# WilliamYi96/HGR-Net

Hardware: AMD Instinct MI355X
Metric: images/sec over 21K-class hierarchy, batch 512; hit@1 parity vs reference (higher is better)
Workload: dtype f16

## Files before the change

### hgr-net_amd/_lib.py

```python
from __future__ import annotations

import ctypes as C
import os
from pathlib import Path

import torch

_HERE = Path(__file__).resolve().parent
LIB_PATH = Path(os.environ.get("HGR_LIB", _HERE / "lib" / "libhgr.so"))

HGR_BF16, HGR_F16 = 0, 1
EPI_NONE, EPI_BIAS, EPI_BIAS_QUICKGELU, EPI_BIAS_RESIDUAL, EPI_BIAS_RELU, EPI_BIAS_ADD16_RELU, EPI_ACCUM, EPI_QGELU_GRAD16 = 0, 1, 2, 3, 4, 5, 6, 7

_p, _i, _l, _f = C.c_void_p, C.c_int, C.c_int64, C.c_float

SIGNATURES = {
    "hgr_gemm_nt": [_p, _l, _p, _l, _p, _l, _p, _p, _l, _i, _i, _i, _i, _i, _i, _p],
    "hgr_gemm_set_tile": [_i],
    "hgr_gemm_set_tail": [_i, _i],
    "hgr_gemm_set_persist": [_i],
    "hgr_gemm_set_ws": [_i],
    "hgr_gemm_set_p8": [_i],
    "hgr_im2col_patches": [_p, _p, _i, _i, _i, _i, _i, _p],
    "hgr_im2col_patches_ex": [_p, _p, _i, _i, _i, _i, _i, _i, _i, _p],
# ... 47 lines not shown
    "hgr_gemm_tn_splitk": [_p, _l, _p, _l, _p, _l, _i, _i, _i, _i, _i, _p],
    "hgr_gemm_tn_tile": [_i, _i],
    "hgr_conv3x3_wgrad_splitk": [_p, _l, _p, _p, _l, _i, _i, _i, _i, _i, _i, _i, _p],
    "hgr_relu_bwd16": [_p, _p, _p, _l, _i, _p],
    "hgr_add16": [_p, _p, _p, _l, _i, _p],
    "hgr_avgpool2_bwd_nhwc": [_p, _p, _i, _i, _i, _i, _i, _p],
    "hgr_attnpool_tokens_bwd": [_p, _p, _i, _i, _i, _i, _p],
    "hgr_im2col3x3_t": [_p, _p, _i, _i, _i, _i, _l, _i, _p],
    "hgr_bn_fold": [_p, _p, _p, _p, _p, _f, _p, _p, _i, _i, _i, _i, _i, _p],
    "hgr_bn_unfold_grad": [_p, _l, _p, _p, _p, _p, _p, _f, _p, _p, _p, _i, _i, _i, _p],
    "hgr_csr_group_aggregate": [_p, _l, _p, _p, _p, _p, _i, _p, _p, _p, _p, _i, _p, _p, _p, _p, _i, _p, _p, _l, _i, _f, _i, _p],
    "hgr_gemm_nt_res_stats": [_p, _l, _p, _l, _p, _p, _l, _p, _p, _i, _i, _i, _i, _p],
    "hgr_vit_head": [_p, _p, _l, _l, _p, _p, _f, _p, _p, _i, _i, _i, _i, _p],
    "hgr_gemm_nt_res_stats_guard": [_p, _l, _p, _l, _p, _p, _l, _p, _p, _f, _p, _i, _i, _i, _i, _p],
    "hgr_gemm_nt_ln": [_p, _l, _p, _l, _p, _l, _p, _p, _p, _f, _i, _i, _i, _i, _i, _p],
    "hgr_gemm_nt_ln_mha": [_p, _l, _p, _l, _p, _p, _p, _f, _p, _l, _i, _i, _i, _i, _i, _p],
    "hgr_gemm_nt_bias_gelu_dual": [_p, _l, _p, _l, _p, _l, _p, _l, _p, _i, _i, _i, _i, _p],
    "hgr_gemm_nt_qgelu_grad_colsum": [_p, _l, _p, _l, _p, _l, _p, _l, _p, _i, _i, _i, _i, _p],
    "hgr_vit_embed_ln_stats": [_p, _p, _p, _p, _p, _p, _p, _p, _i, _i, _i, _f, _i, _p],
    "hgr_row_stats16": [_p, _p, _p, _p, _i, _i, _i, _p],
    "hgr_pair_rows_f32": [_p, _p, _p, _i, _i, _l, _p, _i, _p],
    "hgr_logits_eval_workspace_bytes": [_i, _i],
    "hgr_logits_eval": [_p, _p, _i, _i, _i, _p, _p, _p, _i, _p, _p, _i, _p, _i, _i, _p, _p, _p, _p, _i, _p],
    "hgr_logits_eval_tile_stage": [_p, _p, _i, _i, _i, _p, _p, _p, _i, _p, _p, _i, _p, _i, _i, _p, _p, _p, _p, _i, _p],
    "hgr_logits_eval_row_stage": [_p, _p, _i, _i, _i, _p, _p, _p, _i, _p, _p, _i, _p, _i, _i, _p, _p, _p, _p, _i, _p],
    "hgr_comm_unique_id": [_p],
    "hgr_comm_init": [_i, _i, _p],
    "hgr_comm_destroy": [],
    "hgr_comm_rank": [],
    "hgr_comm_world": [],
# ... 60 lines not shown
```

### hgr-net_amd/clip/model.py

```python
from __future__ import annotations

import os
from collections import OrderedDict
from typing import Dict, Optional, Tuple, Union

import numpy as np
import torch
from torch import nn

from .. import ops
from .._lib import (EPI_BIAS, EPI_BIAS_ADD16_RELU, EPI_BIAS_QUICKGELU, EPI_BIAS_RELU, EPI_BIAS_RESIDUAL, EPI_NONE,
                    HgrError)


class QuickGELU(nn.Module):
    """Placeholder so ``mlp`` keeps the reference's child names (c_fc, gelu, c_proj); the activation
    itself is fused into the c_fc GEMM epilogue (HGR_EPI_BIAS_QUICKGELU)."""


class ResidualAttentionBlock(nn.Module):
    def __init__(self, d_model: int, n_head: int):
        super().__init__()
        self.attn = nn.MultiheadAttention(d_model, n_head)
        self.ln_1 = nn.LayerNorm(d_model)
# ... 117 lines not shown
    def get(self, name: str, shape, dtype, device) -> torch.Tensor:
        n = int(np.prod(shape))
        t = self._b.get(name)
        if t is None or t.numel() < n or t.dtype != dtype or t.device != device:
            t = torch.empty(n, dtype=dtype, device=device)
            self._b[name] = t
            self.epoch += 1
        return t[:n].view(*shape)


IMG_STREAMS = max(1, int(os.environ.get("HGR_IMG_STREAMS", "1")))
IMG_STREAMS_MIN_ROWS = 8192
CLS_LAST = os.environ.get("HGR_CLS_LAST", "1") != "0"
LN_FUSED = os.environ.get("HGR_LN_FUSED", "1") != "0"
QKV_MHA = os.environ.get("HGR_QKV_MHA", "1") != "0"


def ln_fusable(w: int, m: int = 0) -> bool:
    return LN_FUSED and w % 128 == 0 and m * 4 * w * 2 < 2 ** 32


def _run_blocks(x: Optional[torch.Tensor], blocks, heads: int, b: int, l: int, causal: bool, dt: torch.dtype, ws: _Workspace, tag: str,
                taps: Optional[dict] = None, tap_prefix: str = "", pair=None, stats: Optional[torch.Tensor] = None,
                flag: Optional[torch.Tensor] = None, cls_only_last: bool = False):
    m, w = (pair[0] if pair is not None else x).shape
    dev = (pair[0] if pair is not None else x).device
    qkv = ws.get(tag + ".qkv", (m, 3 * w), dt, dev)
    att = ws.get(tag + ".att", (m, w), dt, dev)
    u16 = ws.get(tag + ".u16", (m, 4 * w), dt, dev)
    if pair is not None:
# ... 11 lines not shown
                ops.gemm_nt_ln(ch, k.wf_in[:w], qkv.view(b, l, 3 * w)[:, 0, :w], k.s_in[:w], k.c_in[:w], st_q, k.eps1, tag="q_cls")
            elif fused_attn:
                ops.gemm_nt_ln_mha(xh, k.wf_in, att, k.s_in, k.c_in, stats, b, l, heads, causal, k.eps1)
            else:
                ops.gemm_nt_ln(xh, k.wf_in, qkv, k.s_in, k.c_in, stats, k.eps1, tag="qkv")
            if not fused_attn:
                ops.mha(qkv, att, b, l, heads, causal, q_rows=1 if last_cls else 0)
            if last_cls:
                ca = att.view(b, l, w)[:, 0, :]
                st_c = ws.get(tag + ".stats_cls", (b, w // 64, 2), torch.float32, dev)
                u_c = ws.get(tag + ".u16_cls", (b, 4 * w), dt, dev)
                ops.gemm_nt_res_stats(ca, k.w_out, ch, cl, k.b_out, st_c, tag="out_cls", flag=flag)
                ops.gemm_nt_ln(ch, k.wf_fc, u_c, k.s_fc, k.c_fc, st_c, k.eps2, quickgelu=True, tag="fc_cls")
                ops.gemm_nt_res_stats(u_c, k.w_proj, ch, cl, k.b_proj, st_c, tag="proj_cls", flag=flag)
                break
            ops.gemm_nt_res_stats(att, k.w_out, xh, xl, k.b_out, stats, tag="out", flag=flag)
            ops.gemm_nt_ln(xh, k.wf_fc, u16, k.s_fc, k.c_fc, stats, k.eps2, quickgelu=True, tag="fc")
            ops.gemm_nt_res_stats(u16, k.w_proj, xh, xl, k.b_proj, stats, tag="proj", flag=flag)
            if taps is not None:
                taps[f"{tap_prefix}.resblocks.{i}"] = ops.pair_value(xh, xl).view(b, l, w)
        return None
    h16 = ws.get(tag + ".h16", (m, w), dt, dev)
    for i, k in enumerate(blocks):
        ops.layernorm(x, k.ln1[0], k.ln1[1], h16)
        ops.gemm_nt(h16, k.w_in, qkv, bias=k.b_in, epilogue=EPI_BIAS)
        ops.mha(qkv, att, b, l, heads, causal)
        ops.gemm_nt(att, k.w_out, x, bias=k.b_out, residual=x, epilogue=EPI_BIAS_RESIDUAL)
        ops.layernorm(x, k.ln2[0], k.ln2[1], h16)
        ops.gemm_nt(h16, k.w_fc, u16, bias=k.b_fc, epilogue=EPI_BIAS_QUICKGELU)
        ops.gemm_nt(u16, k.w_proj, x, bias=k.b_proj, residual=x, epilogue=EPI_BIAS_RESIDUAL)
        if taps is not None:
            taps[f"{tap_prefix}.resblocks.{i}"] = x.view(b, l, w).clone()
    return x
# ... 407 lines not shown
```

### hgr-net_amd/csrc/hgr_common.h

```cpp
#pragma once
#include <hip/hip_runtime.h>
#include <stdint.h>
#include <stdio.h>
#include <stdarg.h>
#include <stdlib.h>

#include "../../include/hgr.h"

#define HGR_WAVE 64

#ifdef HGR_LAB
#define HGR_LAB_ON(expr) (expr)
static inline int hgr_lab_env(const char *name) { const char *e = getenv(name); return e ? atoi(e) : 0; }
#else
#define HGR_LAB_ON(expr) false
static inline int hgr_lab_env(const char *) { return 0; }
#endif

typedef __attribute__((ext_vector_type(8))) __bf16 bf16x8;
typedef __attribute__((ext_vector_type(8))) _Float16 f16x8;
typedef __attribute__((ext_vector_type(4))) __bf16 bf16x4;
typedef __attribute__((ext_vector_type(4))) _Float16 f16x4;
typedef __attribute__((ext_vector_type(4))) float f32x4;
typedef __attribute__((ext_vector_type(16))) float f32x16;
typedef __attribute__((ext_vector_type(4))) unsigned int u32x4;
typedef __attribute__((ext_vector_type(2))) unsigned int u32x2;

#define AS1 __attribute__((address_space(1)))
#define AS3 __attribute__((address_space(3)))

template <int DT> struct T16;
template <> struct T16<HGR_BF16> {
    typedef __bf16 elem;
    typedef bf16x8 vec8;
    typedef bf16x4 vec4;
    static __device__ __forceinline__ f32x4 mfma16(vec8 a, vec8 b, f32x4 c) {
        return __builtin_amdgcn_mfma_f32_16x16x32_bf16(a, b, c, 0, 0, 0);
    }
    static __device__ __forceinline__ f32x16 mfma32(vec8 a, vec8 b, f32x16 c) {
        return __builtin_amdgcn_mfma_f32_32x32x16_bf16(a, b, c, 0, 0, 0);
    }
};
template <> struct T16<HGR_F16> {
    typedef _Float16 elem;
// ... 136 lines not shown
```

### hgr-net_amd/csrc/hgr_gemm.hip

```cpp
#include "hgr_gemm_common.h"

using namespace hgr_gemm;

int hgr_conv3x3_c32_launch(const void *x, const void *w, const float *bias, void *out, int B, int H, int W, int Cout, int Kp,
                           int dtype, int relu, void *stream, int pool, int C);

namespace {
constexpr int BM = 128, BN = 128;

int duo_group_env() {
    static int g = -1;
    if (g < 0) { const char *e = getenv("HGR_GEMM_GROUP"); g = e ? atoi(e) : 0; if (g < 0) g = 0; }
    return g;
}
int duo_group() { return duo_group_env() ? duo_group_env() : 4; }
int duo_group_for(int tiles_n) { return duo_group_env() ? duo_group_env() : (tiles_n <= 8 ? 1 : 4); }
int duo_dbg() {
    static int d = -1;
    if (d < 0) d = hgr_lab_env("HGR_GEMM_DBG");
    return d;
}

struct DuoPlan { int big_panels, nbig, tiles_m_half, grid; };
int tail_env = -2, pb_env = -2;
// ... 353 lines not shown
        HGR_CHECK_LAUNCH("hgr_gemm_nt_ln");
        return HGR_OK;
    }
    if (ws_enabled() && hgr_gemm_force_tile() == 0 && ws_covers(M, N, K, WS_LNC)) {
        launch_ws(a, dtype, WS_LNC, act, false, (hipStream_t)stream);
        HGR_CHECK_LAUNCH("hgr_gemm_nt_ln");
        return HGR_OK;
    }
    dim3 grid;
    duo_apply_plan(a, true, grid);
    launch_duo(a, dtype, act ? HGR_EPI_BIAS_QUICKGELU : HGR_EPI_BIAS, false, 2, grid, (hipStream_t)stream);
    HGR_CHECK_LAUNCH("hgr_gemm_nt_ln");
    return HGR_OK;
}

extern "C" int hgr_gemm_nt_bias_gelu_dual(const void *A, int64_t lda, const void *W, int64_t ldw, void *pre, int64_t ldpre, void *post, int64_t ldpost,
                                          const float *bias, int M, int N, int K, int dtype, void *stream) {
    if (int rc = ln_common_checks("hgr_gemm_nt_bias_gelu_dual", A, lda, W, ldw, M, N, K, dtype)) return rc;
    HGR_REQUIRE(pre && post && bias, "hgr_gemm_nt_bias_gelu_dual: null pre / post / bias");
    HGR_REQUIRE(ldpre >= N && ldpost >= N && ldpre % 8 == 0 && ldpost % 8 == 0 && ldpre < (1 << 23) && ldpost < (1 << 23) && hgr_aligned(pre, 16) && hgr_aligned(post, 16) && hgr_aligned(bias, 16),
                "hgr_gemm_nt_bias_gelu_dual: pre / post / bias must be 16-byte aligned, leading dimensions >= N, %% 8 == 0, < 2^23");
    GemmArgs a;
    ln_args(a, A, lda, W, ldw, pre, ldpre, M, N, K);
    a.bias = bias; a.ln_xh = post; a.ln_ldx = ldpost;
    dim3 grid;
    duo_apply_plan(a, true, grid);
    launch_duo(a, dtype, HGR_EPI_BIAS, false, 4, grid, (hipStream_t)stream);
    HGR_CHECK_LAUNCH("hgr_gemm_nt_bias_gelu_dual");
    return HGR_OK;
}
// ... 68 lines not shown
```

### hgr-net_amd/csrc/hgr_gemm_common.h

```cpp
#pragma once
#include "hgr_common.h"
#include <stdlib.h>
#include <type_traits>

namespace hgr_gemm {

constexpr int BK = 64;

struct GemmArgs {
    const char *A; int64_t lda;
    const char *W; int64_t ldw;
    void *C; int64_t ldc;
    const float *bias;
    const float *res; int64_t ldr;
    int M, N, K;
    int tiles_m, tiles_n;
    int m_fastest;
    int vec_ok;
    int dbg;
    int cH, cW, cC, cStride, cHo, cWo;
    unsigned cMagic;
    int cUni;
    int kc; int64_t csplit;
    float *ln_stats; int ln_slots; float ln_eps;
// ... 206 lines not shown
        if constexpr (DW > 0) __builtin_amdgcn_sched_group_barrier(0x200, DW, 0);
        if constexpr (DV > 0) __builtin_amdgcn_sched_group_barrier(0x020, DV, 0);
        mfma16_interleave_step<NR, NW, NV, M_ + 1, NM>();
    }
}
template <int NR, int NW, int NV>
__device__ __forceinline__ void mfma16_interleave() { mfma16_interleave_step<NR, NW, NV, 0>(); }
template <int NR, int NW, int NV>
__device__ __forceinline__ void mfma8_interleave() { mfma16_interleave_step<NR, NW, NV, 0, 8>(); }

enum { V128_PLAIN = 0, V128_TALL = 1, V128_CONV = 2, V128_CONV_TALL = 3 };
void launch_128(const GemmArgs &a, int dtype, int epi, bool out32, int variant, dim3 grid, hipStream_t s);
void launch_256(const GemmArgs &a, int dtype, int epi, bool out32, bool conv, dim3 grid, hipStream_t s);
void launch_duo(const GemmArgs &a, int dtype, int epi, bool out32, int ln, dim3 grid, hipStream_t s);
int duo_set_persist(int enabled);
enum { WS_PLAIN = 0, WS_LNC = 1, WS_LNP = 2 };
bool ws_covers(int M, int N, int K, int mode);
void launch_ws(const GemmArgs &a, int dtype, int mode, int act, bool hasb, hipStream_t s);
int ws_enabled();
int ws_set(int enabled);
bool p8_covers(int M, int N, int K);
void launch_p8(const GemmArgs &a, int dtype, int act, hipStream_t s);
bool p8_wanted(int M, int N, int K);
int p8_set(int mode);

struct SlabArgs {
    const char *A; int64_t lda;
    const char *W; int64_t ldw;
    int M, K, Np;
    const int *tpos, *epos;
// ... 9 lines not shown
```

### hgr-net_amd/csrc/hgr_gemm_duo.hip

```cpp
#include "hgr_gemm_common.h"

namespace hgr_gemm {

#ifndef HGR_PAIR_V2
#define HGR_PAIR_V2 1
#endif
constexpr int NTD = 256;
constexpr int DUO_A0 = 0, DUO_A1 = 32768, DUO_W0 = 65536, DUO_W1 = 73728, DUO_LDS = 81920;

__device__ __forceinline__ void store16_sc1(void *ptr, u32x4 v) {
    asm volatile("global_store_dwordx4 %0, %1, off sc1\n\ts_nop 1" ::"v"(ptr), "v"(v) : "memory");
}

template <int DT, int EPI, bool OUT32, int LN, int MH, bool CONV = false>
__device__ __forceinline__ void duo_tile(const GemmArgs &p, char *smem, const int m0, const int n0) {
    typedef typename T16<DT>::vec8 vec8;
    typedef typename T16<DT>::elem E;
    constexpr int WR = 64 * MH;
    int tid = threadIdx.x;
    if (LN == 1) asm volatile("" : "+v"(tid));
    const int lane = tid & 63;
    const int wave = __builtin_amdgcn_readfirstlane(tid >> 6);
    const int wm = wave >> 1, wn = wave & 1;
    const int r = lane & 15, g = lane >> 4;

    unsigned oA0[4], oA1[4], oW0[2], oW1[2];
    unsigned vA0[CONV ? 4 : 1], vA1[CONV ? 4 : 1];
#pragma unroll
    for (int i = 0; i < 4; ++i) {
        const int id = (i * 4 + wave) * 64 + lane;
        const int pr = id >> 3, c = (id & 7) ^ (pr & 7);
        const int ra = MH == 2 ? (pr >> 6) * 128 + (pr & 63) : pr;
        if (CONV) {
#pragma unroll
            for (int half = 0; half < 2; ++half) {
// ... 82 lines not shown
                for (int i = 0; i < p.ln_slots / 2; ++i) { const f32x4 t = sp[i]; s1 += t[0] + t[2]; s2 += t[1] + t[3]; }
        }
        return ln_finalize(s1, s2, 1.0f / (float)p.K, p.ln_eps);
    };
    const int nk = p.K / 64;
    const int offA = (wm * 64 + r) * 128;
    const int offW = (wn * 32 + r) * 128;
    const int sw0 = ((0 + g) ^ (r & 7)) * 16, sw1 = ((4 + g) ^ (r & 7)) * 16;
    vec8 af[4][2], wf0[2][2], wf1[2][2];
#ifndef HGR_DUO_PF
#define HGR_DUO_PF 2
#endif
#ifndef HGR_DUO_PF_DMA_FIRST
#define HGR_DUO_PF_DMA_FIRST 0
#endif
    constexpr bool PF_BUILD = HGR_DUO_PF == 1 || (HGR_DUO_PF == 2 && LN == 2);
    const bool pf_tile = MH == 2 && !CONV && PF_BUILD && m0 + 256 <= p.M && n0 + 128 <= p.N && (p.K & 127) == 0 && p.K >= 256;
    if (pf_tile) {
      if constexpr (MH == 2 && !CONV && PF_BUILD) {
        vec8 afB[4][2];
        auto &afA = af;
        auto rdW = [&](vec8 (&wf)[2][2], int base) {
#pragma unroll
            for (int j = 0; j < 2; ++j) {
                wf[j][0] = *(const vec8 *)(smem + base + offW + j * 2048 + sw0);
                wf[j][1] = *(const vec8 *)(smem + base + offW + j * 2048 + sw1);
            }
        };
        auto rdA = [&](vec8 (&a)[4][2], int base) {
#pragma unroll
            for (int i = 0; i < 4; ++i) {
// ... 288 lines not shown
            const unsigned gl = (unsigned)rr * ldgB + ch * 16;
#pragma unroll
            for (int q = 0; q < 8 * MH; ++q) {
                const u32x4 v = *(const u32x4 *)(my + (q * 8 + rr) * RS + ch * 16);
                *(u32x4 *)(cw + (cl + q * 8 * ldcB)) = v;
                const vec8 h = __builtin_bit_cast(vec8, v);
                vec8 o;
#pragma unroll
                for (int e = 0; e < 8; ++e) o[e] = quick_gelu_train16<DT>((float)h[e]);
                *(u32x4 *)(gw + (gl + q * 8 * ldgB)) = __builtin_bit_cast(u32x4, o);
            }
            return;
        }
#pragma unroll
        for (int q = 0; q < 8 * MH; ++q)
            *(u32x4 *)(cw + (cl + q * 8 * ldcB)) = *(const u32x4 *)(my + (q * 8 + rr) * RS + ch * 16);
        return;
    }
    if (full && !OUT32 && epi_has_idn16(EPI) && (p.ldc & 7) == 0 && (p.ldr & 7) == 0 && (reinterpret_cast<uintptr_t>(p.C) & 15) == 0 && (reinterpret_cast<uintptr_t>(p.res) & 15) == 0) {
        constexpr int RS = 272;
        char *my = smem + wave * (32 * RS);
        f32x4 bq[2][2];
#pragma unroll
        for (int b = 0; b < 2; ++b)
#pragma unroll
            for (int j = 0; j < 2; ++j) bq[b][j] = HAS_BIAS ? *(const f32x4 *)(p.bias + n0 + wn * 64 + b * 32 + j * 16 + g * 4) : (f32x4){0.f, 0.f, 0.f, 0.f};
        const int r8 = lane >> 3, c8 = lane & 7;
        const int64_t wrow = m0 + wm * WR, wcol = n0 + wn * 64;
        char *cw = (char *)p.C + (wrow * p.ldc + wcol) * 2;
        const char *iw = (const char *)p.res + (wrow * p.ldr + wcol) * 2;
        const unsigned ldcB = (unsigned)p.ldc * 2u, ldiB = (unsigned)p.ldr * 2u;
// ... 120 lines not shown
                        v[e + 4] = (hi4[e] + b8hi[e]) + pair_dec<DT>(oh[e + 4], (ol[1] >> (8 * e)) & 255u);
                    }
#endif
#if HGR_PAIR_V2
                    u32x4 nh;
                    u32x2 nl;
                    {
                        unsigned tq[8];
#pragma unroll
                        for (int e2 = 0; e2 < 4; ++e2) nh[e2] = pair_split2<DT>(v[2 * e2], v[2 * e2 + 1], tq[2 * e2], tq[2 * e2 + 1]);
                        unsigned n0, n1;
                        pair_put_q<DT, 0>(n0, tq[0]); pair_put_q<DT, 1>(n0, tq[1]); pair_put_q<DT, 2>(n0, tq[2]); pair_put_q<DT, 3>(n0, tq[3]);
                        pair_put_q<DT, 0>(n1, tq[4]); pair_put_q<DT, 1>(n1, tq[5]); pair_put_q<DT, 2>(n1, tq[6]); pair_put_q<DT, 3>(n1, tq[7]);
                        nl = (u32x2){n0, n1};
                    }
                    *(u32x4 *)(hw + (xo + (rl + q * 8) * ldxB)) = nh;
#else
                    vec8 nh;
                    u32x2 nl = (u32x2){0u, 0u};
#pragma unroll
                    for (int e = 0; e < 4; ++e) {
                        unsigned q0, q1;
                        E h0, h1;
                        pair_split<DT>(v[e], h0, q0);
                        pair_split<DT>(v[e + 4], h1, q1);
                        nh[e] = h0; nh[e + 4] = h1;
                        nl[0] |= q0 << (8 * e);
                        nl[1] |= q1 << (8 * e);
                    }
                    *(u32x4 *)(hw + (xo + (rl + q * 8) * ldxB)) = __builtin_bit_cast(u32x4, nh);
#endif
                    if (!HGR_LAB_ON(p.dbg & 64)) *(u32x2 *)(lw + (lo8 + (rl + q * 8) * ldlB)) = nl;
                    s1[q] = ((v[0] + v[1]) + (v[2] + v[3])) + ((v[4] + v[5]) + (v[6] + v[7]));
                    s2[q] = (__builtin_fmaf(v[0], v[0], v[1] * v[1]) + __builtin_fmaf(v[2], v[2], v[3] * v[3])) +
                            (__builtin_fmaf(v[4], v[4], v[5] * v[5]) + __builtin_fmaf(v[6], v[6], v[7] * v[7]));
                }
                if (HGR_LAB_ON(p.dbg & 32)) continue;
#define HGR_DPP_STAGE8(CTRL) _Pragma("unroll") for (int q = 0; q < 2; ++q) { \
                    s1[q] += __builtin_bit_cast(float, __builtin_amdgcn_update_dpp(0, __builtin_bit_cast(int, s1[q]), CTRL, 0xF, 0xF, true)); \
                    s2[q] += __builtin_bit_cast(float, __builtin_amdgcn_update_dpp(0, __builtin_bit_cast(int, s2[q]), CTRL, 0xF, 0xF, true)); }
                HGR_DPP_STAGE8(0xB1) HGR_DPP_STAGE8(0x4E) HGR_DPP_STAGE8(0x141)
#undef HGR_DPP_STAGE8
                if (c8 == 0) {
#pragma unroll
                    for (int q = 0; q < 2; ++q) {
                        *(float2 *)(sw + (so + (rl + q * 8) * ldsB)) = make_float2(s1[q], s2[q]);
                        gbits = max(gbits, __float_as_uint(s2[q]));
                    }
                }
            }
            if (p.ln_flag && gbits > __float_as_uint(p.ln_guard)) atomicMax(p.ln_flag, gbits);
            return;
        }
        const float *addp = EPI == HGR_EPI_ACCUM ? (const float *)p.C : p.res;
        const int64_t ldadd = EPI == HGR_EPI_ACCUM ? p.ldc : p.ldr;
        char *cw = (char *)p.C + (wrow * p.ldc + wcol) * 4;
        const char *aw = (const char *)addp + (wrow * ldadd + wcol) * 4;
        const unsigned ldcB = (unsigned)p.ldc * 4u, ldaB = (unsigned)ldadd * 4u;
        const unsigned cl = rq * ldcB + cq * 16, al = rq * ldaB + cq * 16;
#pragma unroll
        for (int a = 0; a < MH; ++a)
// ... 33 lines not shown
        lnrow[tid] = ln_row_stats();
        __syncthreads();
#pragma unroll
        for (int a = 0; a < MH; ++a)
#pragma unroll
        for (int i = 0; i < 4; ++i) {
            const int m = m0 + wm * WR + a * 64 + i * 16 + r;
            const float2 mr = lnrow[wm * WR + a * 64 + i * 16 + r];
            if (m >= p.M) continue;
#pragma unroll
            for (int b = 0; b < 2; ++b)
#pragma unroll
            for (int j = 0; j < 2; ++j) {
                const int n = n0 + wn * 64 + b * 32 + j * 16 + g * 4;
                const f32x4 sq = *(const f32x4 *)(p.ln_s + n), cq4 = *(const f32x4 *)(p.ln_c + n);
                *(u32x2 *)((E *)p.C + (int64_t)m * p.ldc + n) = ln_out16<DT, EPI == HGR_EPI_BIAS_QUICKGELU>(mr, acc[a][b][i][j], sq, cq4);
            }
        }
        return;
    }
    if (LN == 1) {
        typedef typename T16<DT>::vec4 hvec4;
        constexpr int RS = 272;
        char *my = smem + wave * (32 * RS);
        const int rq = lane >> 4, cq = lane & 15;
#pragma unroll
        for (int a = 0; a < MH; ++a)
#pragma unroll
        for (int ih = 0; ih < 2; ++ih) {
            const int row0 = m0 + wm * WR + a * 64 + ih * 32;
#pragma unroll
// ... 11 lines not shown
                const bool ok = row < p.M;
                const int64_t at = row * p.ln_ldx + n0 + wn * 64 + cq * 4;
                if (ok) {
                    const hvec4 oh = *(const hvec4 *)((const E *)p.ln_xh + at);
                    const unsigned ol = *(const unsigned *)((const unsigned char *)p.ln_xl + at);
#pragma unroll
                    for (int e = 0; e < 4; ++e) v[e] += pair_dec<DT>(oh[e], (ol >> (8 * e)) & 255u);
                }
                const float s1 = row16_sum((v[0] + v[1]) + (v[2] + v[3]));
                const float s2 = row16_sum(__builtin_fmaf(v[0], v[0], v[1] * v[1]) + __builtin_fmaf(v[2], v[2], v[3] * v[3]));
                if (ok) {
                    hvec4 nh;
                    unsigned nl = 0u;
#pragma unroll
                    for (int e = 0; e < 4; ++e) { unsigned q; E h; pair_split<DT>(v[e], h, q); nh[e] = h; nl |= q << (8 * e); }
                    *(hvec4 *)((E *)p.ln_xh + at) = nh;
                    *(unsigned *)((unsigned char *)p.ln_xl + at) = nl;
                    if (cq == 0) *(float2 *)(p.ln_stats + (row * p.ln_slots + (n0 >> 6) + wn) * 2) = make_float2(s1, s2);
                    if (cq == 0 && p.ln_flag && __float_as_uint(s2) > __float_as_uint(p.ln_guard)) atomicMax(p.ln_flag, __float_as_uint(s2));
                }
            }
        }
        return;
    }
    if (LN == 4) {
#pragma unroll
        for (int a = 0; a < MH; ++a)
#pragma unroll
        for (int i = 0; i < 4; ++i) {
            const int m = m0 + wm * WR + a * 64 + i * 16 + r;
            if (m >= p.M) continue;
#pragma unroll
            for (int b = 0; b < 2; ++b)
// ... 94 lines not shown
        const int per = GROUP * p.tiles_n, grp = wg / per, first = grp * GROUP;
        const int gs = min(GROUP, tiles_m - first), loc = wg - grp * per;
        tm = first + loc % gs; tn = loc / gs;
    }
    if (half) duo_tile<DT, EPI, OUT32, LN, 1, CONV>(p, smem, p.big_panels * 256 + tm * 128, tn * 128);
    else duo_tile<DT, EPI, OUT32, LN, 2, CONV>(p, smem, tm * 256, tn * 128);
  };
    if constexpr (PERSIST) {
        for (int vb = (int)blockIdx.x; vb < total; vb += (int)gridDim.x) {
            one_tile(vb);
            if (vb + (int)gridDim.x < total) HGR_RBAR();
        }
    } else one_tile((int)blockIdx.x);
}

namespace {
template <int DT>
void launch_duo_dt(const GemmArgs &a, int epi, bool out32, int ln, dim3 grid, hipStream_t s) {
    switch (ln) {
        case 1: hipLaunchKernelGGL((gemm_nt_duo<DT, HGR_EPI_BIAS_RESIDUAL, true, 1>), grid, dim3(NTD), 0, s, a); return;
        case 2:
            if (epi == HGR_EPI_BIAS_QUICKGELU) hipLaunchKernelGGL((gemm_nt_duo<DT, HGR_EPI_BIAS_QUICKGELU, false, 2>), grid, dim3(NTD), 0, s, a);
            else hipLaunchKernelGGL((gemm_nt_duo<DT, HGR_EPI_BIAS, false, 2>), grid, dim3(NTD), 0, s, a);
            return;
        case 4: hipLaunchKernelGGL((gemm_nt_duo<DT, HGR_EPI_BIAS, false, 4>), grid, dim3(NTD), 0, s, a); return;
        case 5: hipLaunchKernelGGL((gemm_nt_duo<DT, HGR_EPI_BIAS_RELU, false, 0, true>), grid, dim3(NTD), 0, s, a); return;
        default: break;
    }
#define HGR_DUO(E) do { if (out32) hipLaunchKernelGGL((gemm_nt_duo<DT, E, true>), grid, dim3(NTD), 0, s, a); \
                        else hipLaunchKernelGGL((gemm_nt_duo<DT, E, false>), grid, dim3(NTD), 0, s, a); } while (0)
// ... 26 lines not shown
        n &= ~7;
        if (n < 8) n = 8;
    }
    return n;
}

void launch_duo(const GemmArgs &a0, int dtype, int epi, bool out32, int ln, dim3 grid, hipStream_t s) {
    GemmArgs a = a0;
    a.total = 0;
    const int ds = duo_slots();
    if (duo_persist() && ln == 1 && grid.y == 1 && !a.kc && (int)grid.x > ds && (int)grid.x <= 2 * ds) { a.total = (int)grid.x; grid.x = (unsigned)ds; }
    if (dtype == HGR_BF16) launch_duo_dt<HGR_BF16>(a, epi, out32, ln, grid, s);
    else launch_duo_dt<HGR_F16>(a, epi, out32, ln, grid, s);
}

}
```

### hgr-net_amd/ops.py

```python
from __future__ import annotations

from typing import Optional

import torch

from . import _lib
from ._lib import (EPI_ACCUM, EPI_BIAS, EPI_BIAS_ADD16_RELU, EPI_BIAS_QUICKGELU, EPI_BIAS_RELU, EPI_BIAS_RESIDUAL, EPI_NONE, EPI_QGELU_GRAD16,
                   HGR_BF16, HGR_F16)

PROFILE = None

WEIGHTS_GEN = [0]

SPLIT_HOOK = None


def split_point(name: str) -> None:
    h = SPLIT_HOOK
    if h is not None:
        h(name)


TORCH16 = {HGR_BF16: torch.bfloat16, HGR_F16: torch.float16}
PAIR_LO = torch.uint8
# ... 104 lines not shown
def gelu_dual_ok(m: int, n: int, k: int, lda: int, ldw: int) -> bool:
    return n % 128 == 0 and k % 64 == 0 and k >= 128 and m * lda * 2 < (1 << 32) and n * ldw * 2 < (1 << 32)


def gemm_nt_ln(x16: torch.Tensor, wfold: torch.Tensor, out: torch.Tensor, ln_s: torch.Tensor, ln_c: torch.Tensor, stats: torch.Tensor,
               eps: float = 1e-5, quickgelu: bool = False, tag: str = "") -> torch.Tensor:
    m, k = x16.shape
    n = wfold.shape[0]
    assert x16.dtype == wfold.dtype == out.dtype and out.shape[0] == m and out.shape[1] >= n and ln_s.numel() == n and ln_c.numel() == n
    assert x16.stride(1) == wfold.stride(1) == out.stride(1) == 1 and stats.dtype == torch.float32 and stats.numel() >= m * (k // 64) * 2
    ev = _prof_begin()
    _lib.call("hgr_gemm_nt_ln", _dev(x16), x16.stride(0), _dev(wfold), wfold.stride(0), _dev(out), out.stride(0), _dev(ln_s), _dev(ln_c),
              _dev(stats), float(eps), m, n, k, DT_OF[x16.dtype], 1 if quickgelu else 0, _stream())
    _prof_end(ev, 2.0 * m * n * k, 2 * m * k + 2 * n * k + 2 * m * n, tag)
    return out


def gemm_nt_ln_mha(x16: torch.Tensor, wfold: torch.Tensor, att: torch.Tensor, ln_s: torch.Tensor, ln_c: torch.Tensor, stats: torch.Tensor,
                   b: int, l: int, heads: int, causal: bool, eps: float = 1e-5, tag: str = "qkv_mha") -> torch.Tensor:
    m, k = x16.shape
    w = heads * 64
    assert m == b * l and k == w and wfold.shape == (3 * w, k) and x16.dtype == wfold.dtype == att.dtype and att.shape == (m, w)
    assert x16.stride(1) == wfold.stride(1) == att.stride(1) == 1 and ln_s.numel() == ln_c.numel() == 3 * w
    assert stats.dtype == torch.float32 and stats.numel() >= m * (k // 64) * 2
    ev = _prof_begin()
    _lib.call("hgr_gemm_nt_ln_mha", _dev(x16), x16.stride(0), _dev(wfold), wfold.stride(0), _dev(ln_s), _dev(ln_c), _dev(stats), float(eps),
              _dev(att), att.stride(0), b, l, heads, 1 if causal else 0, DT_OF[x16.dtype], _stream())
    _prof_end(ev, 2.0 * m * 3 * w * k + 4.0 * b * heads * l * l * 64, 2 * m * k + 2 * 3 * w * k + 2 * m * w, tag)
    return att

# ... 638 lines not shown
```

### include/hgr.h

```cpp
#ifndef HGR_H
#define HGR_H

#include <stdint.h>

#ifdef __cplusplus
extern "C" {
#endif

#define HGR_ABI_VERSION 4

enum { HGR_OK = 0, HGR_EINVAL = -1, HGR_EUNSUPPORTED = -2, HGR_ELAUNCH = -3 };

typedef enum { HGR_BF16 = 0, HGR_F16 = 1 } hgr_dtype_t;

typedef enum {
    HGR_EPI_NONE = 0,
    HGR_EPI_BIAS = 1,
    HGR_EPI_BIAS_QUICKGELU = 2,
    HGR_EPI_BIAS_RESIDUAL = 3,
    HGR_EPI_BIAS_RELU = 4,
    HGR_EPI_BIAS_ADD16_RELU = 5,
    HGR_EPI_ACCUM = 6,
    HGR_EPI_QGELU_GRAD16 = 7
} hgr_epilogue_t;
// ... 161 lines not shown
int hgr_adamw(float *p, const float *g, float *m, float *v, int64_t n, float lr, float beta1, float beta2, float eps,
              float wd, int step, const float *sumsq_total, float max_norm, float grad_scale, void *stream);

int hgr_gemm_nt_res_stats(const void *A, int64_t lda, const void *W, int64_t ldw, void *xh, void *xl, int64_t ldx,
                          const float *bias, float *stats, int M, int N, int K, int dtype, void *stream);

int hgr_gemm_nt_res_stats_guard(const void *A, int64_t lda, const void *W, int64_t ldw, void *xh, void *xl, int64_t ldx,
                                const float *bias, float *stats, float guard_sumsq, uint32_t *flag,
                                int M, int N, int K, int dtype, void *stream);

int hgr_vit_head(const void *xh, const void *xl, int64_t ldx, int64_t row_mul, const float *gamma, const float *beta, float eps,
                 const void *proj_t, float *out, int B, int W, int D, int dtype, void *stream);
int hgr_gemm_nt_ln(const void *XH, int64_t ldx, const void *Wfold, int64_t ldw, void *C, int64_t ldc,
                   const float *ln_s, const float *ln_c, const float *stats, float eps,
                   int M, int N, int K, int dtype, int act, void *stream);

int hgr_gemm_nt_ln_mha(const void *XH, int64_t ldx, const void *Wfold, int64_t ldw, const float *ln_s, const float *ln_c,
                       const float *stats, float eps, void *att, int64_t ldatt, int B, int L, int heads, int causal,
                       int dtype, void *stream);

int hgr_gemm_nt_bias_gelu_dual(const void *A, int64_t lda, const void *W, int64_t ldw, void *pre, int64_t ldpre, void *post, int64_t ldpost,
                               const float *bias, int M, int N, int K, int dtype, void *stream);
int hgr_gemm_nt_qgelu_grad_colsum(const void *A, int64_t lda, const void *W, int64_t ldw, void *C, int64_t ldc, const void *pre, int64_t ldpre,
                                  float *colsum_part, int M, int N, int K, int dtype, void *stream);
int hgr_vit_embed_ln_stats(const float *patches, const float *class_embedding, const float *positional_embedding,
                           const float *gamma, const float *beta, void *xh, void *xl, float *stats,
                           int B, int G, int W, float eps, int dtype, void *stream);
int hgr_row_stats16(const float *x, void *xh, void *xl, float *stats, int rows, int W, int dtype, void *stream);
int hgr_pair_rows_f32(const void *xh, const void *xl, float *out, int rows, int W, int64_t row_mul, const int32_t *row_idx, int dtype, void *stream);

// ... 35 lines not shown
```

Before: 110,100.

## Fuse out-proj, MLP fc and proj GEMMs into one persistent chained kernel

Replaces the three per-block launches (attention out-projection with residual and stats, LN-folded fc with QuickGELU, and MLP projection with residual) with one persistent kernel. Blocks pull tiles from per-XCD atomic queues, and per-row-panel counters let a later phase start on a panel as soon as its inputs are complete. The aim is to remove launch gaps and tail idle time between dependent GEMMs by overlapping phases across row panels. In exchange it adds spin-wait polling, sc1 write-through stores, disabled prefetch paths in the chained tiles, and a workspace that must be reset, with a risk of stalls if scheduling is poor.

```diff
diff --git a/hgr-net_amd/_lib.py b/hgr-net_amd/_lib.py
--- a/hgr-net_amd/_lib.py
+++ b/hgr-net_amd/_lib.py
@@ -85,6 +85,8 @@
     "hgr_vit_head": [_p, _p, _l, _l, _p, _p, _f, _p, _p, _i, _i, _i, _i, _p],
     "hgr_gemm_nt_res_stats_guard": [_p, _l, _p, _l, _p, _p, _l, _p, _p, _f, _p, _i, _i, _i, _i, _p],
     "hgr_gemm_nt_ln": [_p, _l, _p, _l, _p, _l, _p, _p, _p, _f, _i, _i, _i, _i, _i, _p],
+    "hgr_gemm_chain_out_mlp": [_p, _l, _p, _p, _p, _p, _l, _p, _f, _p, _p, _p, _p, _f, _p, _l, _p, _p, _p, _l, _i, _i, _i, _p],
+    "hgr_gemm_chain_workspace_bytes": [_i],
     "hgr_gemm_nt_ln_mha": [_p, _l, _p, _l, _p, _p, _p, _f, _p, _l, _i, _i, _i, _i, _i, _p],
     "hgr_gemm_nt_bias_gelu_dual": [_p, _l, _p, _l, _p, _l, _p, _l, _p, _i, _i, _i, _i, _p],
     "hgr_gemm_nt_qgelu_grad_colsum": [_p, _l, _p, _l, _p, _l, _p, _l, _p, _i, _i, _i, _i, _p],
diff --git a/hgr-net_amd/clip/model.py b/hgr-net_amd/clip/model.py
--- a/hgr-net_amd/clip/model.py
+++ b/hgr-net_amd/clip/model.py
@@ -155,6 +155,7 @@
 CLS_LAST = os.environ.get("HGR_CLS_LAST", "1") != "0"
 LN_FUSED = os.environ.get("HGR_LN_FUSED", "1") != "0"
 QKV_MHA = os.environ.get("HGR_QKV_MHA", "1") != "0"
+MLP_CHAIN = os.environ.get("HGR_MLP_CHAIN", "1") != "0"
 
 
 def ln_fusable(w: int, m: int = 0) -> bool:
@@ -196,9 +197,13 @@
                 ops.gemm_nt_ln(ch, k.wf_fc, u_c, k.s_fc, k.c_fc, st_c, k.eps2, quickgelu=True, tag="fc_cls")
                 ops.gemm_nt_res_stats(u_c, k.w_proj, ch, cl, k.b_proj, st_c, tag="proj_cls", flag=flag)
                 break
-            ops.gemm_nt_res_stats(att, k.w_out, xh, xl, k.b_out, stats, tag="out", flag=flag)
-            ops.gemm_nt_ln(xh, k.wf_fc, u16, k.s_fc, k.c_fc, stats, k.eps2, quickgelu=True, tag="fc")
-            ops.gemm_nt_res_stats(u16, k.w_proj, xh, xl, k.b_proj, stats, tag="proj", flag=flag)
+            if MLP_CHAIN and ops.chain_ok(m, w, xh.stride(0)):
+                work = ws.const(f"{tag}.chain_work.{m}", lambda: ops.chain_work(m, dev))
+                ops.gemm_chain_out_mlp(att, k.w_out, k.b_out, xh, xl, stats, k.wf_fc, k.s_fc, k.c_fc, k.eps2, u16, k.w_proj, k.b_proj, work, flag=flag)
+            else:
+                ops.gemm_nt_res_stats(att, k.w_out, xh, xl, k.b_out, stats, tag="out", flag=flag)
+                ops.gemm_nt_ln(xh, k.wf_fc, u16, k.s_fc, k.c_fc, stats, k.eps2, quickgelu=True, tag="fc")
+                ops.gemm_nt_res_stats(u16, k.w_proj, xh, xl, k.b_proj, stats, tag="proj", flag=flag)
             if taps is not None:
                 taps[f"{tap_prefix}.resblocks.{i}"] = ops.pair_value(xh, xl).view(b, l, w)
         return None
diff --git a/hgr-net_amd/csrc/hgr_common.h b/hgr-net_amd/csrc/hgr_common.h
--- a/hgr-net_amd/csrc/hgr_common.h
+++ b/hgr-net_amd/csrc/hgr_common.h
@@ -28,6 +28,7 @@
 
 #define AS1 __attribute__((address_space(1)))
 #define AS3 __attribute__((address_space(3)))
+#define AS4 __attribute__((address_space(4)))
 
 template <int DT> struct T16;
 template <> struct T16<HGR_BF16> {
diff --git a/hgr-net_amd/csrc/hgr_gemm.hip b/hgr-net_amd/csrc/hgr_gemm.hip
--- a/hgr-net_amd/csrc/hgr_gemm.hip
+++ b/hgr-net_amd/csrc/hgr_gemm.hip
@@ -391,6 +391,44 @@
     return HGR_OK;
 }
 
+extern "C" int64_t hgr_gemm_chain_workspace_bytes(int M) {
+    return M < 1 ? 0 : 4 * ((int64_t)HGR_CHAIN_PANEL + (M + 127) / 128);
+}
+
+extern "C" int hgr_gemm_chain_out_mlp(const void *att, int64_t ldatt, const void *w_out, const float *b_out,
+                                      void *xh, void *xl, int64_t ldx, float *stats, float guard_sumsq, uint32_t *flag,
+                                      const void *w_fc, const float *ln_s, const float *ln_c, float eps, void *u16, int64_t ldu,
+                                      const void *w_proj, const float *b_proj, void *work, int64_t work_bytes,
+                                      int M, int W, int dtype, void *stream) {
+    const char *who = "hgr_gemm_chain_out_mlp";
+    if (int rc = ln_common_checks(who, att, ldatt, w_out, W, M, W, W, dtype)) return rc;
+    if (int rc = ln_common_checks(who, xh, ldx, w_fc, W, M, 4 * W, W, dtype)) return rc;
+    if (int rc = ln_common_checks(who, u16, ldu, w_proj, 4 * W, M, W, 4 * W, dtype)) return rc;
+    HGR_REQUIRE(W % 128 == 0, "%s: the row width W=%d must be a multiple of 128", who, W);
+    HGR_REQUIRE(xl && b_out && b_proj && stats && ln_s && ln_c, "%s: null xl / b_out / b_proj / stats / ln_s / ln_c", who);
+    HGR_REQUIRE(!flag || (guard_sumsq > 0.f && hgr_aligned(flag, 4)), "%s: flag needs guard_sumsq > 0 and 4-byte alignment", who);
+    HGR_REQUIRE(ldx >= W && ldx % 8 == 0 && ldx < (1 << 23) && hgr_aligned(xh, 16) && hgr_aligned(xl, 16), "%s: xh / xl must be 16-byte aligned, ldx %% 8 == 0, ldx < 2^23", who);
+    HGR_REQUIRE(ldu >= 4 * W && ldu % 8 == 0 && ldu < (1 << 23) && hgr_aligned(u16, 16), "%s: u16 must be 16-byte aligned with ldu >= 4 W, ldu %% 8 == 0, ldu < 2^23", who);
+    HGR_REQUIRE(hgr_aligned(b_out, 16) && hgr_aligned(b_proj, 16) && hgr_aligned(ln_s, 16) && hgr_aligned(ln_c, 16) && hgr_aligned(stats, 16),
+                "%s: b_out / b_proj / ln_s / ln_c / stats must be 16-byte aligned", who);
+    HGR_REQUIRE(work && hgr_aligned(work, 16) && work_bytes >= hgr_gemm_chain_workspace_bytes(M), "%s: work must be 16-byte aligned with at least %lld bytes",
+                who, (long long)hgr_gemm_chain_workspace_bytes(M));
+    ChainArgs c;
+    GemmArgs &o = c.g[0], &f = c.g[1], &pj = c.g[2];
+    ln_args(o, att, ldatt, w_out, W, nullptr, 0, M, W, W);
+    o.bias = b_out; o.ln_stats = stats; o.ln_slots = W / 64; o.ln_xh = xh; o.ln_xl = xl; o.ln_ldx = ldx; o.ln_flag = flag; o.ln_guard = guard_sumsq;
+    o.group = duo_group_for(o.tiles_n);
+    ln_args(f, xh, ldx, w_fc, W, u16, ldu, M, 4 * W, W);
+    f.ln_stats = stats; f.ln_slots = W / 64; f.ln_eps = eps; f.ln_s = ln_s; f.ln_c = ln_c;
+    f.group = duo_group_for(f.tiles_n);
+    pj = o;
+    pj.A = (const char *)u16; pj.lda = ldu; pj.W = (const char *)w_proj; pj.ldw = 4 * W; pj.K = 4 * W; pj.bias = b_proj;
+    c.work = (unsigned *)work; c.units = (M + 127) / 128;
+    launch_chain(c, dtype, (hipStream_t)stream);
+    HGR_CHECK_LAUNCH("hgr_gemm_chain_out_mlp");
+    return HGR_OK;
+}
+
 extern "C" int hgr_gemm_nt_bias_gelu_dual(const void *A, int64_t lda, const void *W, int64_t ldw, void *pre, int64_t ldpre, void *post, int64_t ldpost,
                                           const float *bias, int M, int N, int K, int dtype, void *stream) {
     if (int rc = ln_common_checks("hgr_gemm_nt_bias_gelu_dual", A, lda, W, ldw, M, N, K, dtype)) return rc;
diff --git a/hgr-net_amd/csrc/hgr_gemm_common.h b/hgr-net_amd/csrc/hgr_gemm_common.h
--- a/hgr-net_amd/csrc/hgr_gemm_common.h
+++ b/hgr-net_amd/csrc/hgr_gemm_common.h
@@ -244,6 +244,9 @@
 void launch_256(const GemmArgs &a, int dtype, int epi, bool out32, bool conv, dim3 grid, hipStream_t s);
 void launch_duo(const GemmArgs &a, int dtype, int epi, bool out32, int ln, dim3 grid, hipStream_t s);
 int duo_set_persist(int enabled);
+struct ChainArgs { GemmArgs g[3]; unsigned *work; int units; };
+enum { HGR_CHAIN_QUEUE = 0, HGR_CHAIN_DONE = 256, HGR_CHAIN_ERR = 288, HGR_CHAIN_PANEL = 320 };
+void launch_chain(const ChainArgs &c, int dtype, hipStream_t s);
 enum { WS_PLAIN = 0, WS_LNC = 1, WS_LNP = 2 };
 bool ws_covers(int M, int N, int K, int mode);
 void launch_ws(const GemmArgs &a, int dtype, int mode, int act, bool hasb, hipStream_t s);
diff --git a/hgr-net_amd/csrc/hgr_gemm_duo.hip b/hgr-net_amd/csrc/hgr_gemm_duo.hip
--- a/hgr-net_amd/csrc/hgr_gemm_duo.hip
+++ b/hgr-net_amd/csrc/hgr_gemm_duo.hip
@@ -12,13 +12,24 @@
     asm volatile("global_store_dwordx4 %0, %1, off sc1\n\ts_nop 1" ::"v"(ptr), "v"(v) : "memory");
 }
 
-template <int DT, int EPI, bool OUT32, int LN, int MH, bool CONV = false>
+template <bool SC1, class T>
+__device__ __forceinline__ void st_out(void *ptr, const T &v) {
+    if constexpr (!SC1) *(T *)ptr = v;
+    else if constexpr (sizeof(T) == 16) store16_sc1(ptr, __builtin_bit_cast(u32x4, v));
+    else if constexpr (sizeof(T) == 8) asm volatile("global_store_dwordx2 %0, %1, off sc1\n\ts_nop 1" ::"v"(ptr), "v"(__builtin_bit_cast(u32x2, v)) : "memory");
+    else {
+        static_assert(sizeof(T) == 4, "st_out: 4, 8 or 16 bytes");
+        asm volatile("global_store_dword %0, %1, off sc1\n\ts_nop 1" ::"v"(ptr), "v"(__builtin_bit_cast(unsigned, v)) : "memory");
+    }
+}
+
+template <int DT, int EPI, bool OUT32, int LN, int MH, bool CONV = false, bool SC1 = false>
 __device__ __forceinline__ void duo_tile(const GemmArgs &p, char *smem, const int m0, const int n0) {
     typedef typename T16<DT>::vec8 vec8;
     typedef typename T16<DT>::elem E;
     constexpr int WR = 64 * MH;
     int tid = threadIdx.x;
-    if (LN == 1) asm volatile("" : "+v"(tid));
+    if (LN == 1 || SC1) asm volatile("" : "+v"(tid));
     const int lane = tid & 63;
     const int wave = __builtin_amdgcn_readfirstlane(tid >> 6);
     const int wm = wave >> 1, wn = wave & 1;
@@ -131,7 +142,7 @@
 #ifndef HGR_DUO_PF_DMA_FIRST
 #define HGR_DUO_PF_DMA_FIRST 0
 #endif
-    constexpr bool PF_BUILD = HGR_DUO_PF == 1 || (HGR_DUO_PF == 2 && LN == 2);
+    constexpr bool PF_BUILD = !SC1 && (HGR_DUO_PF == 1 || (HGR_DUO_PF == 2 && LN == 2));
     const bool pf_tile = MH == 2 && !CONV && PF_BUILD && m0 + 256 <= p.M && n0 + 128 <= p.N && (p.K & 127) == 0 && p.K >= 256;
     if (pf_tile) {
       if constexpr (MH == 2 && !CONV && PF_BUILD) {
@@ -450,7 +461,7 @@
         }
 #pragma unroll
         for (int q = 0; q < 8 * MH; ++q)
-            *(u32x4 *)(cw + (cl + q * 8 * ldcB)) = *(const u32x4 *)(my + (q * 8 + rr) * RS + ch * 16);
+            st_out<SC1>(cw + (cl + q * 8 * ldcB), *(const u32x4 *)(my + (q * 8 + rr) * RS + ch * 16));
         return;
     }
     if (full && !OUT32 && epi_has_idn16(EPI) && (p.ldc & 7) == 0 && (p.ldr & 7) == 0 && (reinterpret_cast<uintptr_t>(p.C) & 15) == 0 && (reinterpret_cast<uintptr_t>(p.res) & 15) == 0) {
@@ -601,7 +612,7 @@
                         pair_put_q<DT, 0>(n1, tq[4]); pair_put_q<DT, 1>(n1, tq[5]); pair_put_q<DT, 2>(n1, tq[6]); pair_put_q<DT, 3>(n1, tq[7]);
                         nl = (u32x2){n0, n1};
                     }
-                    *(u32x4 *)(hw + (xo + (rl + q * 8) * ldxB)) = nh;
+                    st_out<SC1>(hw + (xo + (rl + q * 8) * ldxB), nh);
 #else
                     vec8 nh;
                     u32x2 nl = (u32x2){0u, 0u};
@@ -615,9 +626,9 @@
                         nl[0] |= q0 << (8 * e);
                         nl[1] |= q1 << (8 * e);
                     }
-                    *(u32x4 *)(hw + (xo + (rl + q * 8) * ldxB)) = __builtin_bit_cast(u32x4, nh);
+                    st_out<SC1>(hw + (xo + (rl + q * 8) * ldxB), __builtin_bit_cast(u32x4, nh));
 #endif
-                    if (!HGR_LAB_ON(p.dbg & 64)) *(u32x2 *)(lw + (lo8 + (rl + q * 8) * ldlB)) = nl;
+                    if (!HGR_LAB_ON(p.dbg & 64)) st_out<SC1>(lw + (lo8 + (rl + q * 8) * ldlB), nl);
                     s1[q] = ((v[0] + v[1]) + (v[2] + v[3])) + ((v[4] + v[5]) + (v[6] + v[7]));
                     s2[q] = (__builtin_fmaf(v[0], v[0], v[1] * v[1]) + __builtin_fmaf(v[2], v[2], v[3] * v[3])) +
                             (__builtin_fmaf(v[4], v[4], v[5] * v[5]) + __builtin_fmaf(v[6], v[6], v[7] * v[7]));
@@ -631,7 +642,7 @@
                 if (c8 == 0) {
 #pragma unroll
                     for (int q = 0; q < 2; ++q) {
-                        *(float2 *)(sw + (so + (rl + q * 8) * ldsB)) = make_float2(s1[q], s2[q]);
+                        st_out<SC1>(sw + (so + (rl + q * 8) * ldsB), make_float2(s1[q], s2[q]));
                         gbits = max(gbits, __float_as_uint(s2[q]));
                     }
                 }
@@ -695,7 +706,7 @@
             for (int j = 0; j < 2; ++j) {
                 const int n = n0 + wn * 64 + b * 32 + j * 16 + g * 4;
                 const f32x4 sq = *(const f32x4 *)(p.ln_s + n), cq4 = *(const f32x4 *)(p.ln_c + n);
-                *(u32x2 *)((E *)p.C + (int64_t)m * p.ldc + n) = ln_out16<DT, EPI == HGR_EPI_BIAS_QUICKGELU>(mr, acc[a][b][i][j], sq, cq4);
+                st_out<SC1>((E *)p.C + (int64_t)m * p.ldc + n, ln_out16<DT, EPI == HGR_EPI_BIAS_QUICKGELU>(mr, acc[a][b][i][j], sq, cq4));
             }
         }
         return;
@@ -737,9 +748,9 @@
                     unsigned nl = 0u;
 #pragma unroll
                     for (int e = 0; e < 4; ++e) { unsigned q; E h; pair_split<DT>(v[e], h, q); nh[e] = h; nl |= q << (8 * e); }
-                    *(hvec4 *)((E *)p.ln_xh + at) = nh;
-                    *(unsigned *)((unsigned char *)p.ln_xl + at) = nl;
-                    if (cq == 0) *(float2 *)(p.ln_stats + (row * p.ln_slots + (n0 >> 6) + wn) * 2) = make_float2(s1, s2);
+                    st_out<SC1>((E *)p.ln_xh + at, nh);
+                    st_out<SC1>((unsigned char *)p.ln_xl + at, nl);
+                    if (cq == 0) st_out<SC1>(p.ln_stats + (row * p.ln_slots + (n0 >> 6) + wn) * 2, make_float2(s1, s2));
                     if (cq == 0 && p.ln_flag && __float_as_uint(s2) > __float_as_uint(p.ln_guard)) atomicMax(p.ln_flag, __float_as_uint(s2));
                 }
             }
@@ -864,6 +875,76 @@
     } else one_tile((int)blockIdx.x);
 }
 
+typedef AS1 unsigned chain_u32;
+__device__ __forceinline__ unsigned chain_poll(const chain_u32 *p) {
+    unsigned v;
+    asm volatile("global_load_dword %0, %1, off sc1\n\ts_waitcnt vmcnt(0)" : "=v"(v) : "v"(p) : "memory");
+    return v;
+}
+
+template <int DT>
+__global__ __launch_bounds__(NTD, 2) void gemm_chain_duo(ChainArgs c) {
+    __shared__ __attribute__((aligned(1024))) char smem[DUO_LDS];
+    chain_u32 *const work = (chain_u32 *)c.work;
+    const int tid = threadIdx.x;
+    const int xq = blockIdx.x & 7;
+    const int uq = c.units >> 3, ur = c.units & 7;
+    const int nu = uq + (xq < ur ? 1 : 0), u0 = xq * uq + min(xq, ur);
+    const int nfull = nu >> 1, npan = nfull + (nu & 1);
+    const int tno = c.g[0].N >> 7, tnf = c.g[1].N >> 7;
+    const int e0 = npan * tno, e1 = e0 + npan * tnf, e2 = e1 + npan * tno;
+    chain_u32 *const queue = work + HGR_CHAIN_QUEUE + xq * 32;
+    int *const tk = (int *)smem;
+    if (tid == 0) tk[0] = (int)__hip_atomic_fetch_add(queue, 1u, __ATOMIC_RELAXED, __HIP_MEMORY_SCOPE_AGENT);
+    for (;;) {
+        HGR_RBAR();
+        const int t = __builtin_amdgcn_readfirstlane(tk[0]);
+        if (t >= e2) break;
+        unsigned nxt = 0u;
+        if (tid == 0) nxt = __hip_atomic_fetch_add(queue, 1u, __ATOMIC_RELAXED, __HIP_MEMORY_SCOPE_AGENT);
+        const int ph = t < e0 ? 0 : (t < e1 ? 1 : 2);
+        const int loc = t - (ph == 0 ? 0 : (ph == 1 ? e0 : e1));
+        const int tnp = ph == 1 ? tnf : tno, G = c.g[ph].group;
+        const int per = G * tnp, grp = loc / per, first = grp * G, gs = min(G, npan - first), l2 = loc - grp * per;
+        const int pm = first + l2 % gs, tn = l2 / gs;
+        const int unit = u0 + 2 * pm;
+        chain_u32 *const ctr = work + HGR_CHAIN_PANEL + unit;
+        if (ph && tid == 0) {
+            const unsigned need = (unsigned)(ph == 1 ? tno : tno + tnf);
+            for (unsigned spins = 0; chain_poll(ctr) < need;) {
+                __builtin_amdgcn_s_sleep(2);
+                if (++spins == (1u << 22)) { st_out<true>((void *)(work + HGR_CHAIN_ERR), 1u); break; }
+            }
+            __builtin_amdgcn_fence(__ATOMIC_ACQUIRE, "agent");
+            asm volatile("s_waitcnt vmcnt(0)" ::: "memory");
+        }
+        HGR_RBAR();
+        const int m0 = unit * 128, n0 = tn * 128;
+        const char AS4 *ka = (const char AS4 *)__builtin_amdgcn_kernarg_segment_ptr();
+        asm volatile("" : "+s"(ka));
+        const GemmArgs &p = *(const GemmArgs *)(ka + offsetof(ChainArgs, g) + ph * sizeof(GemmArgs));
+        if (ph == 1) {
+            if (pm >= nfull) duo_tile<DT, HGR_EPI_BIAS_QUICKGELU, false, 2, 1, false, true>(p, smem, m0, n0);
+            else duo_tile<DT, HGR_EPI_BIAS_QUICKGELU, false, 2, 2, false, true>(p, smem, m0, n0);
+        } else {
+            if (pm >= nfull) duo_tile<DT, HGR_EPI_BIAS_RESIDUAL, true, 1, 1, false, true>(p, smem, m0, n0);
+            else duo_tile<DT, HGR_EPI_BIAS_RESIDUAL, true, 1, 2, false, true>(p, smem, m0, n0);
+        }
+        asm volatile("s_waitcnt vmcnt(0)" ::: "memory");
+        HGR_RBAR();
+        if (tid == 0) {
+            __hip_atomic_fetch_add(ctr, 1u, __ATOMIC_RELAXED, __HIP_MEMORY_SCOPE_AGENT);
+            tk[0] = (int)nxt;
+        }
+    }
+    asm volatile("s_waitcnt vmcnt(0)" ::: "memory");
+    if (tid == 0) tk[1] = __hip_atomic_fetch_add(work + HGR_CHAIN_DONE, 1u, __ATOMIC_RELAXED, __HIP_MEMORY_SCOPE_AGENT) == gridDim.x - 1u;
+    HGR_RBAR();
+    if (tk[1])
+        for (int i = tid; i < HGR_CHAIN_PANEL + c.units; i += NTD)
+            if (i != HGR_CHAIN_ERR) st_out<true>((void *)(work + i), 0u);
+}
+
 namespace {
 template <int DT>
 void launch_duo_dt(const GemmArgs &a, int epi, bool out32, int ln, dim3 grid, hipStream_t s) {
@@ -920,4 +1001,10 @@
     else launch_duo_dt<HGR_F16>(a, epi, out32, ln, grid, s);
 }
 
-}
+void launch_chain(const ChainArgs &c, int dtype, hipStream_t s) {
+    const dim3 grid((unsigned)duo_slots());
+    if (dtype == HGR_BF16) hipLaunchKernelGGL(gemm_chain_duo<HGR_BF16>, grid, dim3(NTD), 0, s, c);
+    else hipLaunchKernelGGL(gemm_chain_duo<HGR_F16>, grid, dim3(NTD), 0, s, c);
+}
+
+}
diff --git a/hgr-net_amd/ops.py b/hgr-net_amd/ops.py
--- a/hgr-net_amd/ops.py
+++ b/hgr-net_amd/ops.py
@@ -142,6 +142,36 @@
               _dev(stats), float(eps), m, n, k, DT_OF[x16.dtype], 1 if quickgelu else 0, _stream())
     _prof_end(ev, 2.0 * m * n * k, 2 * m * k + 2 * n * k + 2 * m * n, tag)
     return out
+
+
+def chain_ok(m: int, w: int, ldx: Optional[int] = None) -> bool:
+    ldx = w if ldx is None else ldx
+    return m >= 1 and w >= 128 and w % 128 == 0 and ldx >= w and ldx % 8 == 0 and ldx < (1 << 23) and m * 4 * w * 2 < (1 << 32) and m * ldx * 2 < (1 << 32)
+
+
+def chain_work(m: int, device) -> torch.Tensor:
+    n = int(_lib.load().hgr_gemm_chain_workspace_bytes(m))
+    return torch.zeros((n + 15) // 16 * 4, dtype=torch.int32, device=device)
+
+
+def gemm_chain_out_mlp(att: torch.Tensor, w_out: torch.Tensor, b_out: torch.Tensor, xh: torch.Tensor, xl: torch.Tensor, stats: torch.Tensor,
+                       wf_fc: torch.Tensor, s_fc: torch.Tensor, c_fc: torch.Tensor, eps: float, u16: torch.Tensor, w_proj: torch.Tensor,
+                       b_proj: torch.Tensor, work: torch.Tensor, flag: Optional[torch.Tensor] = None, tag: str = "out_mlp") -> None:
+    m, w = xh.shape
+    assert att.shape == (m, w) and w_out.shape == (w, w) and wf_fc.shape == (4 * w, w) and w_proj.shape == (w, 4 * w)
+    assert u16.shape[0] == m and u16.shape[1] >= 4 * w and xl.dtype == PAIR_LO and xh.shape == xl.shape and xh.stride() == xl.stride()
+    assert att.dtype == w_out.dtype == xh.dtype == wf_fc.dtype == u16.dtype == w_proj.dtype
+    assert w_out.is_contiguous() and wf_fc.is_contiguous() and w_proj.is_contiguous() and att.stride(1) == xh.stride(1) == u16.stride(1) == 1
+    assert stats.dtype == torch.float32 and stats.numel() >= m * (w // 64) * 2 and s_fc.numel() == c_fc.numel() == 4 * w
+    if flag is not None:
+        assert flag.numel() == 1 and flag.element_size() == 4
+    ev = _prof_begin()
+    _lib.call("hgr_gemm_chain_out_mlp", _dev(att), att.stride(0), _dev(w_out), _dev(b_out), _dev(xh), _dev(xl), xh.stride(0), _dev(stats),
+              LN_GUARD_SUMSQ if flag is not None else 0.0, _dev(flag), _dev(wf_fc), _dev(s_fc), _dev(c_fc), float(eps), _dev(u16), u16.stride(0),
+              _dev(w_proj), _dev(b_proj), _dev(work), work.numel() * work.element_size(), m, w, DT_OF[xh.dtype], _stream())
+    st = 8 * m * (w // 64)
+    _prof_end(ev, 18.0 * m * w * w,
+              (2 * m * w + 2 * w * w + 6 * m * w + st) + (2 * m * w + 8 * w * w + 8 * m * w) + (8 * m * w + 8 * w * w + 6 * m * w + st), tag)
 
 
 def gemm_nt_ln_mha(x16: torch.Tensor, wfold: torch.Tensor, att: torch.Tensor, ln_s: torch.Tensor, ln_c: torch.Tensor, stats: torch.Tensor,
diff --git a/include/hgr.h b/include/hgr.h
--- a/include/hgr.h
+++ b/include/hgr.h
@@ -199,6 +199,13 @@
 int hgr_gemm_nt_ln(const void *XH, int64_t ldx, const void *Wfold, int64_t ldw, void *C, int64_t ldc,
                    const float *ln_s, const float *ln_c, const float *stats, float eps,
                    int M, int N, int K, int dtype, int act, void *stream);
+
+int hgr_gemm_chain_out_mlp(const void *att, int64_t ldatt, const void *w_out, const float *b_out,
+                           void *xh, void *xl, int64_t ldx, float *stats, float guard_sumsq, uint32_t *flag,
+                           const void *w_fc, const float *ln_s, const float *ln_c, float eps, void *u16, int64_t ldu,
+                           const void *w_proj, const float *b_proj, void *work, int64_t work_bytes,
+                           int M, int W, int dtype, void *stream);
+int64_t hgr_gemm_chain_workspace_bytes(int M);
 
 int hgr_gemm_nt_ln_mha(const void *XH, int64_t ldx, const void *Wfold, int64_t ldw, const float *ln_s, const float *ln_c,
                        const float *stats, float eps, void *att, int64_t ldatt, int B, int L, int heads, int causal,
```

New measurement: 100,100 (median of 2 runs). -9.1%, worse.
